# andrew-angus/andvaranaut

Hardware: AMD Instinct MI355X
Metric: gp_lml_evals_per_s (higher is better)
Workload: dtype f64; 1 GPU; Matern52 GP LML eval (assembly + Cholesky + solve), N=16384 d=16, LHS inputs; N=16384, d=16, kernel=Matern52, parallelism=replicas x1 (one chain per GPU)

## Files before the change

andvaranaut_amd/csrc/gemm_f64.hip:

```cpp
#include <cstdlib>
#include <type_traits>
#include "migp_kernels.h"

namespace migp {

typedef double double2_t __attribute__((ext_vector_type(2)));
typedef double double4_t __attribute__((ext_vector_type(4)));

constexpr int TILE = 128;
constexpr int LDS_LD = 144;

__device__ __forceinline__ void tile_from_index(int tri, int nt, int idx, int& ti, int& tj) {
  if (tri) {
    const int ntri = nt * (nt + 1) / 2;
    if (idx < ntri) {
      int t = (int)((sqrt(8.0 * (double)idx + 1.0) - 1.0) * 0.5);
      while ((t + 1) * (t + 2) / 2 <= idx) ++t;
      while (t * (t + 1) / 2 > idx) --t;
      ti = t;
      tj = idx - t * (t + 1) / 2;
    } else {
      const int rem = idx - ntri;
      ti = nt + rem / nt;
      tj = rem % nt;
    }
  } else {
    ti = idx / nt;
    tj = idx % nt;
  }
}
__device__ __forceinline__ void tile_from_index(const GemmParams& p, int idx, int& ti, int& tj) {
  tile_from_index(p.tri, p.nt, idx, ti, tj);
}

__device__ __forceinline__ void tile_from_index_banded(int tri, int mt, int nt, int idx, int R, int& ti, int& tj) {
  auto before = [&](int r) {
    if (!tri) return r * nt;
    return r <= nt ? r * (r + 1) / 2 : nt * (nt + 1) / 2 + (r - nt) * nt;
  };
  int lo = 0, hi = (mt + R - 1) / R - 1;
  while (lo < hi) {
    const int mid = (lo + hi + 1) >> 1;
    if (before(mid * R) <= idx) lo = mid; else hi = mid - 1;
  }
  const int r0 = lo * R, r1 = min(r0 + R, mt), h = r1 - r0;
  int e = idx - before(r0);
  const int cfull = tri ? min(r0 + 1, nt) : nt;
  if (e < cfull * h) { tj = e / h; ti = r0 + e % h; return; }
  e -= cfull * h;
  for (tj = cfull; tj < nt; ++tj) {
    const int cnt = r1 - tj;
    if (e < cnt) { ti = tj + e; return; }
    e -= cnt;
  }
  ti = r1 - 1; tj = min(ti, nt - 1);
}

__device__ __forceinline__ void tile_from_index_banded(const GemmParams& p, int idx, int R, int& ti, int& tj) {
  tile_from_index_banded(p.tri, p.mt, p.nt, idx, R, ti, tj);
}

__device__ __forceinline__ void tile_from_index_fc(int mt, int nt, int fc, int band, int idx, int& ti, int& tj) {
  const int ft = fc * (fc + 1) / 2 + (mt - fc) * fc;
  if (idx < ft) {
    tile_from_index(1, fc, idx, ti, tj);
  } else {
    if (band > 0) tile_from_index_banded(1, mt - fc, nt - fc, idx - ft, band, ti, tj);
    else tile_from_index(1, nt - fc, idx - ft, ti, tj);
    ti += fc;
    tj += fc;
  }
}

__device__ __forceinline__ void list_tile(const GemmParams& p, int idx, int& ra, int& rb, int& rc, int& cc, bool& diag) {
  const int want = idx + p.pl[p.pl_first].x;
  int lo = p.pl_first, hi = p.pl_first + p.pl_n - 1;
  while (lo < hi) {
    const int mid = (lo + hi + 1) >> 1;
    if (p.pl[mid].x <= want) lo = mid; else hi = mid - 1;
  }
  const int4 d = p.pl[lo];
  int ti, tj;
  if (p.band > 0) tile_from_index_banded(1, p.pl_rows - d.y, d.w, want - d.x, p.band, ti, tj);
  else tile_from_index(1, d.w, want - d.x, ti, tj);
  ra = d.y - p.pl_abase + ti;
  rb = d.y - p.pl_abase + tj;
  rc = d.y + ti;
  cc = d.z + tj;
  diag = (ti == tj);
}

namespace vb {
constexpr int BKB = 16;
constexpr int OPER_B = BKB * LDS_LD;
constexpr int NT_B = 256;
constexpr int NQB = TILE * BKB / 2 / NT_B;
#ifndef MIGP_SWZ_B
#define MIGP_SWZ_B 0
#endif
constexpr bool SWZ = MIGP_SWZ_B != 0;

template <bool KMAJOR>
__device__ __forceinline__ void chunk_offsets(long ld, int tid, unsigned& goff, unsigned& loff, long& gstride) {
  if (KMAJOR) {
    const int k = tid >> 6, xc = tid & 63;
    goff = (unsigned)((k * ld + 2 * xc) * 8);
    loff = (unsigned)((k * LDS_LD + 2 * xc) * 8);
    gstride = 4 * ld * 8;
  } else if (SWZ) {
    const int kc = tid & 7, row = tid >> 3;
    goff = (unsigned)((row * ld + 2 * kc) * 8);
    loff = (unsigned)(((2 * kc) * LDS_LD + (row ^ (2 * kc))) * 8);
    gstride = 32 * ld * 8;
  } else {
    const int xl = tid & 15, kc = (tid >> 4) & 7, xh = tid >> 7;
    goff = (unsigned)(((xh * 16 + xl) * ld + 2 * kc) * 8);
    loff = (unsigned)(((2 * kc) * LDS_LD + xh * 16 + xl) * 8);
    gstride = 32 * ld * 8;
  }
}
__device__ __forceinline__ void chunk_load(const char* __restrict__ base, unsigned goff, long gstride,
                                           double2_t (&r)[NQB]) {
#pragma unroll
  for (int q = 0; q < NQB; ++q) r[q] = *reinterpret_cast<const double2_t*>(base + q * gstride + goff);
}
template <bool KMAJOR>
__device__ __forceinline__ void chunk_store(char* __restrict__ lds, unsigned loff, const double2_t (&r)[NQB]) {
#pragma unroll
  for (int q = 0; q < NQB; ++q) {
    if (KMAJOR) {
      *reinterpret_cast<double2_t*>(lds + loff + q * (4 * LDS_LD * 8)) = r[q];
    } else {
      *reinterpret_cast<double*>(lds + loff + q * (32 * 8)) = r[q].x;
      *reinterpret_cast<double*>(lds + loff + q * (32 * 8) + LDS_LD * 8) = r[q].y;
    }
  }
}
}

template <bool A_KMAJOR, bool B_KMAJOR>
__global__ __launch_bounds__(vb::NT_B, 2) void gemm_f64_kernel_b(GemmParams p) {
  using vb::BKB; using vb::OPER_B; using vb::NQB;
  extern __shared__ __attribute__((aligned(16))) double smem[];
  double* As = smem;
  double* Bs = smem + 2 * OPER_B;
  const int tid = threadIdx.x;
  const int lane = tid & 63;
  const int wave = tid >> 6;
  const int wr = wave >> 1, wc = wave & 1;

  const int nblk = gridDim.x;
  int idx = blockIdx.x;
  if (p.kmode == 0) {
    const int b = blockIdx.x, x = b & 7, q = nblk >> 3, r = nblk & 7;
    idx = (x < r ? x * (q + 1) : r * (q + 1) + (x - r) * q) + (b >> 3);
  }
  idx += p.tile0;
  int ti, tj;
  int rc, cc;
  if (p.pl) {
    bool diag;
    list_tile(p, idx, ti, tj, rc, cc, diag);
  } else {
    if (p.fc > 0) tile_from_index_fc(p.mt, p.nt, p.fc, p.band, idx, ti, tj);
    else if (p.band > 0 && p.tri && p.kmode == 0) tile_from_index_banded(p, idx, p.band, ti, tj);
    else tile_from_index(p, idx, ti, tj);
    if (p.kmode == 2 && !p.tri) ti = p.mt - 1 - ti;
    if (p.kmode == 4 && !p.tri) { tj = p.nt - 1 - idx / p.mt; ti = idx % p.mt; }
    rc = ti;
    cc = tj;
  }
  const int i0 = ti * TILE, j0 = tj * TILE;
  int kbeg = 0, kend = p.k;
  if (p.kmode == 1) kbeg = j0;
  else if (p.kmode == 2) kend = i0 + TILE;
  else if (p.kmode == 3) kbeg = i0;
  else if (p.kmode == 4) kend = j0 + TILE;

  const long z1 = p.batch1 > 0 ? (long)(blockIdx.z % p.batch1) : (long)blockIdx.z, z2 = p.batch1 > 0 ? (long)(blockIdx.z / p.batch1) : 0;
  const double* A = p.A + z1 * p.strideA + z2 * p.strideA2;
  const double* B = p.B + z1 * p.strideB + z2 * p.strideB2;
  double* C = p.C + z1 * p.strideC + z2 * p.strideC2;

  double4_t acc[4][4];
#pragma unroll
  for (int a = 0; a < 4; ++a)
#pragma unroll
    for (int b = 0; b < 4; ++b) acc[a][b] = (double4_t){0.0, 0.0, 0.0, 0.0};

  const int nchunk = (kend - kbeg) / BKB;
  unsigned gA, lA, gB, lB;
  long sA, sB;
  vb::chunk_offsets<A_KMAJOR>(p.lda, tid, gA, lA, sA);
  vb::chunk_offsets<B_KMAJOR>(p.ldb, tid, gB, lB, sB);
  const char* Ag = reinterpret_cast<const char*>(A_KMAJOR ? A + (long)kbeg * p.lda + i0 : A + (long)i0 * p.lda + kbeg);
  const char* Bg = reinterpret_cast<const char*>(B_KMAJOR ? B + (long)kbeg * p.ldb + j0 : B + (long)j0 * p.ldb + kbeg);
  const long stepA = (A_KMAJOR ? (long)BKB * p.lda : (long)BKB) * 8;
  const long stepB = (B_KMAJOR ? (long)BKB * p.ldb : (long)BKB) * 8;
  const int segmask = p.kseg > 0 ? p.kseg / BKB - 1 : 0x7fffffff;
  const long segjump = (p.kseg_stride - (long)(p.kseg - BKB)) * 8;
  char* Asb = reinterpret_cast<char*>(As);
  char* Bsb = reinterpret_cast<char*>(Bs);
  double2_t ra[2][NQB], rb[2][NQB];
  if (nchunk > 0) {
    vb::chunk_load(Ag, gA, sA, ra[0]);
    vb::chunk_load(Bg, gB, sB, rb[0]);
    if (nchunk > 1) {
      Ag += stepA;
      Bg += stepB;
      vb::chunk_load(Ag, gA, sA, ra[1]);
      vb::chunk_load(Bg, gB, sB, rb[1]);
    }
    vb::chunk_store<A_KMAJOR>(Asb, lA, ra[0]);
    vb::chunk_store<B_KMAJOR>(Bsb, lB, rb[0]);
  }
  __syncthreads();

  const int kq = lane >> 4, l15 = lane & 15;
  const double* a_ptr[4];
  const double* b_ptr[4];
#pragma unroll
  for (int kk = 0; kk < 4; ++kk) {
    const int sa = (vb::SWZ && !A_KMAJOR) ? (4 * kk + (kq & 2)) : 0, sb = (vb::SWZ && !B_KMAJOR) ? (4 * kk + (kq & 2)) : 0;
    a_ptr[kk] = As + kq * LDS_LD + wr * 64 + (l15 ^ sa);
    b_ptr[kk] = Bs + kq * LDS_LD + wc * 64 + (l15 ^ sb);
  }
  double af[2][4], bf[2][4];
  auto load_frags = [&](int set, int boff, int kk) {
    const double* ap = a_ptr[kk] + boff + kk * 4 * LDS_LD;
    const double* bp = b_ptr[kk] + boff + kk * 4 * LDS_LD;
#pragma unroll
    for (int a = 0; a < 4; ++a) af[set][a] = ap[16 * a];
#pragma unroll
    for (int b = 0; b < 4; ++b) bf[set][b] = bp[16 * b];
  };
  if (nchunk > 0) load_frags(0, 0, 0);

  const double alpha = p.alpha, beta = p.beta;
  double* cbase = C + (long)(rc * TILE + wr * 64 + kq) * p.ldc + cc * TILE + wc * 64 + l15;
  double4_t cv[2][4];
  auto load_group = [&](int set, int a) {
#pragma unroll
    for (int b = 0; b < 4; ++b)
#pragma unroll
      for (int r = 0; r < 4; ++r) cv[set][b][r] = cbase[(long)(16 * a + 4 * r) * p.ldc + 16 * b];
  };
  auto chunk_body = [&](int c, auto S, auto LASTC) {
    constexpr int s = decltype(S)::value;
    constexpr int lastc = decltype(LASTC)::value;
    constexpr int boff = s * OPER_B;
    const bool adv = (c + 2 < nchunk);
    const bool seg = ((c + 2) & segmask) == 0;
    Ag += adv ? (seg ? segjump : stepA) : 0;
    Bg += adv ? (seg ? segjump : stepB) : 0;
#pragma unroll
    for (int kk = 0; kk < BKB / 4; ++kk) {
      const int cur = kk & 1;
      __builtin_amdgcn_sched_barrier(0);
      if (kk == 0) {
        if (lastc == 0) {
          vb::chunk_load(Ag, gA, sA, ra[s]);
          vb::chunk_load(Bg, gB, sB, rb[s]);
        } else {
          load_group(lastc - 1, lastc - 1);
        }
      }
      if (kk + 1 < BKB / 4) load_frags(cur ^ 1, boff, kk + 1);
#pragma unroll
      for (int a = 0; a < 4; ++a)
#pragma unroll
        for (int b = 0; b < 4; ++b)
          acc[a][b] = __builtin_amdgcn_mfma_f64_16x16x4f64(af[cur][a], bf[cur][b], acc[a][b], 0, 0, 0);
      if (kk == BKB / 4 - 1) {
        constexpr int noff = (boff ^ OPER_B) * 8;
        vb::chunk_store<A_KMAJOR>(Asb + noff, lA, ra[s ^ 1]);
        vb::chunk_store<B_KMAJOR>(Bsb + noff, lB, rb[s ^ 1]);
      }
      if (kk == 0) {
#pragma unroll
        for (int g = 0; g < 4; ++g) {
          __builtin_amdgcn_sched_group_barrier(0x008, 1, 0);
          __builtin_amdgcn_sched_group_barrier(0x020, 1, 0);
          __builtin_amdgcn_sched_group_barrier(0x008, 1, 0);
          __builtin_amdgcn_sched_group_barrier(0x020, 1, 0);
          __builtin_amdgcn_sched_group_barrier(0x008, 1, 0);
          __builtin_amdgcn_sched_group_barrier(0x100, 1, 0);
          __builtin_amdgcn_sched_group_barrier(0x008, 1, 0);
        }
      } else if (kk + 1 < BKB / 4) {
#pragma unroll
        for (int g = 0; g < 4; ++g) {
          __builtin_amdgcn_sched_group_barrier(0x008, 3, 0);
          __builtin_amdgcn_sched_group_barrier(0x100, 1, 0);
          __builtin_amdgcn_sched_group_barrier(0x008, 1, 0);
        }
      } else {
        constexpr int nw = (A_KMAJOR ? NQB : 2 * NQB) + (B_KMAJOR ? NQB : 2 * NQB);
#pragma unroll
        for (int g = 0; g < 16; ++g) {
          __builtin_amdgcn_sched_group_barrier(0x008, 1, 0);
          if (g < nw) __builtin_amdgcn_sched_group_barrier(0x200, 1, 0);
        }
      }
    }
    __builtin_amdgcn_sched_barrier(0);
    __syncthreads();
    load_frags(0, boff ^ OPER_B, 0);
  };
  int c = 0;
  for (; c + 2 < nchunk; c += 2) {
    chunk_body(c, std::integral_constant<int, 0>(), std::integral_constant<int, 0>());
    chunk_body(c + 1, std::integral_constant<int, 1>(), std::integral_constant<int, 0>());
  }
  chunk_body(c, std::integral_constant<int, 0>(), std::integral_constant<int, 1>());
  chunk_body(c + 1, std::integral_constant<int, 1>(), std::integral_constant<int, 2>());

  if (beta != 0.0) {
#pragma unroll
    for (int a = 0; a < 4; ++a) {
#pragma unroll
      for (int b = 0; b < 4; ++b)
#pragma unroll
        for (int r = 0; r < 4; ++r)
          cbase[(long)(16 * a + 4 * r) * p.ldc + 16 * b] = alpha * acc[a][b][r] + beta * cv[a & 1][b][r];
      if (a + 2 < 4) load_group(a & 1, a + 2);
    }
  } else {
#pragma unroll
    for (int a = 0; a < 4; ++a)
#pragma unroll
      for (int b = 0; b < 4; ++b)
#pragma unroll
        for (int r = 0; r < 4; ++r) cbase[(long)(16 * a + 4 * r) * p.ldc + 16 * b] = alpha * acc[a][b][r];
  }
}

namespace vs {
constexpr int TS = 64;
constexpr int BKS = 16;
constexpr int LDS_S = 80;
constexpr int OPER_S = BKS * LDS_S;
constexpr int NQS = TS * BKS / 2 / 256;
constexpr int NBUF = 3;
#ifndef MIGP_SWZ_S
#define MIGP_SWZ_S 1
#endif
constexpr bool SWZ = MIGP_SWZ_S != 0;
#ifndef MIGP_XCD_MAP_S
#define MIGP_XCD_MAP_S 1
#endif

template <bool KMAJOR>
__device__ __forceinline__ void chunk_offsets(long ld, int tid, unsigned& goff, unsigned& loff, long& gstride) {
  if (KMAJOR) {
    const int k = tid >> 5, xc = tid & 31;
    goff = (unsigned)((k * ld + 2 * xc) * 8);
    loff = (unsigned)((k * LDS_S + 2 * xc) * 8);
    gstride = 8 * ld * 8;
  } else if (SWZ) {
    const int kc = tid & 7, row = tid >> 3;
    goff = (unsigned)((row * ld + 2 * kc) * 8);
    loff = (unsigned)(((2 * kc) * LDS_S + (row ^ (2 * kc))) * 8);
    gstride = 32 * ld * 8;
  } else {
    const int xl = tid & 15, kc = (tid >> 4) & 7, xh = tid >> 7;
    goff = (unsigned)(((xh * 16 + xl) * ld + 2 * kc) * 8);
    loff = (unsigned)(((2 * kc) * LDS_S + xh * 16 + xl) * 8);
    gstride = 32 * ld * 8;
  }
}
__device__ __forceinline__ void chunk_load(const char* __restrict__ base, unsigned goff, long gstride,
                                           double2_t (&r)[NQS]) {
#pragma unroll
  for (int q = 0; q < NQS; ++q) r[q] = *reinterpret_cast<const double2_t*>(base + q * gstride + goff);
}
template <bool KMAJOR>
__device__ __forceinline__ void chunk_store(char* __restrict__ lds, unsigned loff, const double2_t (&r)[NQS]) {
#pragma unroll
  for (int q = 0; q < NQS; ++q) {
    if (KMAJOR) {
      *reinterpret_cast<double2_t*>(lds + loff + q * (8 * LDS_S * 8)) = r[q];
    } else {
      *reinterpret_cast<double*>(lds + loff + q * (32 * 8)) = r[q].x;
      *reinterpret_cast<double*>(lds + loff + q * (32 * 8) + LDS_S * 8) = r[q].y;
    }
  }
}
}

template <bool A_KMAJOR, bool B_KMAJOR, bool FLUSH = false>
__global__ __launch_bounds__(256, 2) void gemm_f64_kernel_s(GemmParams p) {
  using vs::BKS; using vs::OPER_S; using vs::NQS; using vs::LDS_S; using vs::TS;
  if (p.hiprio) __builtin_amdgcn_s_setprio(3);
  __shared__ __attribute__((aligned(16))) double smem[2 * vs::NBUF * vs::OPER_S];
  double* As = smem;
  double* Bs = smem + vs::NBUF * OPER_S;
  const int tid = threadIdx.x;
  const int lane = tid & 63;
  const int wave = tid >> 6;
  const int wr = wave >> 1, wc = wave & 1;

  int ti, tj;
  int rc, cc;
  int bid = (int)blockIdx.x;
  if (MIGP_XCD_MAP_S && p.kmode == 0) {
    const int nblk = (int)gridDim.x, x = bid & 7, q = nblk >> 3, r = nblk & 7;
    bid = (x < r ? x * (q + 1) : r * (q + 1) + (x - r) * q) + (bid >> 3);
  }
  if (p.pl) {
    int ra, rb, prc, pcc;
    bool diag;
    const int quad = bid & 3;
    list_tile(p, p.sub_base + (bid >> 2), ra, rb, prc, pcc, diag);
    if (diag && quad == 1) return;
    ti = 2 * ra + (quad >> 1);
    tj = 2 * rb + (quad & 1);
    rc = 2 * prc + (quad >> 1);
    cc = 2 * pcc + (quad & 1);
  } else {
    if (p.sub_base >= 0) {
      int pti, ptj;
      const int pidx = p.sub_base + (bid >> 2), quad = bid & 3;
      if (p.fc > 0) tile_from_index_fc(p.sub_mt, p.sub_nt, p.fc, p.band, pidx, pti, ptj);
      else if (p.band > 0 && p.tri) tile_from_index_banded(p.tri, p.sub_mt, p.sub_nt, pidx, p.band, pti, ptj);
      else tile_from_index(p.tri, p.sub_nt, pidx, pti, ptj);
      ti = 2 * pti + (quad >> 1);
      tj = 2 * ptj + (quad & 1);
      if (p.tri && tj > ti) return;
      if (p.dead_last_half && ti == 2 * p.sub_mt - 1) return;
    } else {
      tile_from_index(p, bid, ti, tj);
      if (p.dead_last_half && ti == p.mt - 1) return;
    }
    if (p.kmode == 2 && !p.tri) ti = p.mt - 1 - ti;
    if (p.kmode == 4 && !p.tri) { tj = p.nt - 1 - (int)blockIdx.x / p.mt; ti = (int)blockIdx.x % p.mt; }
    rc = ti;
    cc = tj;
  }
  const int i0 = ti * TS, j0 = tj * TS;
  int kbeg = 0, kend = p.k;
  if (p.kmode == 1) kbeg = j0;
  else if (p.kmode == 2) kend = i0 + TS;
  else if (p.kmode == 3) kbeg = i0;
  else if (p.kmode == 4) kend = j0 + TS;
  kbeg &= ~(BKS - 1);

  const long z1 = p.batch1 > 0 ? (long)(blockIdx.z % p.batch1) : (long)blockIdx.z, z2 = p.batch1 > 0 ? (long)(blockIdx.z / p.batch1) : 0;
  const double* A = p.A + z1 * p.strideA + z2 * p.strideA2;
  const double* B = p.B + z1 * p.strideB + z2 * p.strideB2;
  double* C = p.C + z1 * p.strideC + z2 * p.strideC2;

  double4_t acc[2][2];
#pragma unroll
  for (int a = 0; a < 2; ++a)
#pragma unroll
    for (int b = 0; b < 2; ++b) acc[a][b] = (double4_t){0.0, 0.0, 0.0, 0.0};

  const int nchunk = (kend - kbeg) / BKS;
  unsigned gA, lA, gB, lB;
  long sA, sB;
  vs::chunk_offsets<A_KMAJOR>(p.lda, tid, gA, lA, sA);
  vs::chunk_offsets<B_KMAJOR>(p.ldb, tid, gB, lB, sB);
  const char* Ag = reinterpret_cast<const char*>(A_KMAJOR ? A + (long)kbeg * p.lda + i0 : A + (long)i0 * p.lda + kbeg);
  const char* Bg = reinterpret_cast<const char*>(B_KMAJOR ? B + (long)kbeg * p.ldb + j0 : B + (long)j0 * p.ldb + kbeg);
  const long stepA = (A_KMAJOR ? (long)BKS * p.lda : (long)BKS) * 8;
  const long stepB = (B_KMAJOR ? (long)BKS * p.ldb : (long)BKS) * 8;
  const int segmask = p.kseg > 0 ? p.kseg / BKS - 1 : 0x7fffffff;
  const long segjump = (p.kseg_stride - (long)(p.kseg - BKS)) * 8;
  char* Asb = reinterpret_cast<char*>(As);
  char* Bsb = reinterpret_cast<char*>(Bs);
  constexpr int NB = vs::NBUF;
  double2_t ra[NB][NQS], rb[NB][NQS];
  auto advance = [&](int next_chunk) {
    const bool adv = next_chunk < nchunk;
    const bool seg = (next_chunk & segmask) == 0;
    Ag += adv ? (seg ? segjump : stepA) : 0;
    Bg += adv ? (seg ? segjump : stepB) : 0;
  };
  if (nchunk > 0) {
#pragma unroll
    for (int u = 0; u < NB; ++u) {
      vs::chunk_load(Ag, gA, sA, ra[u]);
      vs::chunk_load(Bg, gB, sB, rb[u]);
      advance(u + 1);
    }
    vs::chunk_store<A_KMAJOR>(Asb, lA, ra[0]);
    vs::chunk_store<B_KMAJOR>(Bsb, lB, rb[0]);
    vs::chunk_store<A_KMAJOR>(Asb + OPER_S * 8, lA, ra[1]);
    vs::chunk_store<B_KMAJOR>(Bsb + OPER_S * 8, lB, rb[1]);
    vs::chunk_load(Ag, gA, sA, ra[0]);
    vs::chunk_load(Bg, gB, sB, rb[0]);
    advance(4);
  }
  const int kq = lane >> 4, l15 = lane & 15;
  const double alpha = p.alpha, beta = p.beta;
  double* cbase = C + (long)(rc * TS + wr * 32 + kq) * p.ldc + cc * TS + wc * 32 + l15;
  double4_t cv[2][2];
  if (beta != 0.0) {
#pragma unroll
    for (int a = 0; a < 2; ++a)
#pragma unroll
      for (int b = 0; b < 2; ++b)
#pragma unroll
        for (int r = 0; r < 4; ++r) cv[a][b][r] = cbase[(long)(16 * a + 4 * r) * p.ldc + 16 * b];
  }
  __syncthreads();

  const double* a_ptr[4];
  const double* b_ptr[4];
#pragma unroll
  for (int kk = 0; kk < 4; ++kk) {
    const int sa = (vs::SWZ && !A_KMAJOR) ? (4 * kk + (kq & 2)) : 0, sb = (vs::SWZ && !B_KMAJOR) ? (4 * kk + (kq & 2)) : 0;
    a_ptr[kk] = As + kq * LDS_S + wr * 32 + (l15 ^ sa);
    b_ptr[kk] = Bs + kq * LDS_S + wc * 32 + (l15 ^ sb);
  }
  double fa[2][2], fb[2][2];
  auto load_frags = [&](int set, int boff, int kk) {
    const double* ap = a_ptr[kk] + boff + kk * 4 * LDS_S;
    const double* bp = b_ptr[kk] + boff + kk * 4 * LDS_S;
    fa[set][0] = ap[0]; fa[set][1] = ap[16]; fb[set][0] = bp[0]; fb[set][1] = bp[16];
  };
  if (nchunk > 0) load_frags(0, 0, 0);
  const int kflush_chunks = FLUSH ? p.kflush / BKS : 1;
  auto chunk_body = [&](int c, auto Sc) {
    constexpr int sidx = decltype(Sc)::value;
    constexpr int boff = sidx * OPER_S;
    constexpr int s1 = (sidx + 1) % NB, s2 = (sidx + 2) % NB;
#pragma unroll
    for (int kk = 0; kk < BKS / 4; ++kk) {
      const int cur = kk & 1;
      __builtin_amdgcn_sched_barrier(0);
      if (kk == 0) {
        vs::chunk_load(Ag, gA, sA, ra[s1]);
        vs::chunk_load(Bg, gB, sB, rb[s1]);
      }
      if (kk + 1 < BKS / 4) load_frags(cur ^ 1, boff, kk + 1);
      else load_frags(cur ^ 1, s1 * OPER_S, 0);
      acc[0][0] = __builtin_amdgcn_mfma_f64_16x16x4f64(fa[cur][0], fb[cur][0], acc[0][0], 0, 0, 0);
      acc[0][1] = __builtin_amdgcn_mfma_f64_16x16x4f64(fa[cur][0], fb[cur][1], acc[0][1], 0, 0, 0);
      acc[1][0] = __builtin_amdgcn_mfma_f64_16x16x4f64(fa[cur][1], fb[cur][0], acc[1][0], 0, 0, 0);
      acc[1][1] = __builtin_amdgcn_mfma_f64_16x16x4f64(fa[cur][1], fb[cur][1], acc[1][1], 0, 0, 0);
      if (kk == BKS / 4 - 1) {
        vs::chunk_store<A_KMAJOR>(Asb + s2 * OPER_S * 8, lA, ra[s2]);
        vs::chunk_store<B_KMAJOR>(Bsb + s2 * OPER_S * 8, lB, rb[s2]);
      }
      if (kk == 0) {
#pragma unroll
        for (int g = 0; g < 2; ++g) {
          __builtin_amdgcn_sched_group_barrier(0x008, 1, 0);
          __builtin_amdgcn_sched_group_barrier(0x020, 1, 0);
          __builtin_amdgcn_sched_group_barrier(0x100, 1, 0);
          __builtin_amdgcn_sched_group_barrier(0x008, 1, 0);
          __builtin_amdgcn_sched_group_barrier(0x020, 1, 0);
        }
      } else if (kk + 1 < BKS / 4) {
#pragma unroll
        for (int g = 0; g < 2; ++g) {
          __builtin_amdgcn_sched_group_barrier(0x008, 1, 0);
          __builtin_amdgcn_sched_group_barrier(0x100, 1, 0);
          __builtin_amdgcn_sched_group_barrier(0x008, 1, 0);
        }
      } else {
#pragma unroll
        for (int g = 0; g < 4; ++g) {
          __builtin_amdgcn_sched_group_barrier(0x008, 1, 0);
          __builtin_amdgcn_sched_group_barrier(0x100, 1, 0);
          __builtin_amdgcn_sched_group_barrier(0x200, 2, 0);
        }
      }
    }
    advance(c + 5);
    __builtin_amdgcn_sched_barrier(0);
    if constexpr (FLUSH) if ((c + 1) % kflush_chunks == 0 && c + 1 < nchunk) {
#pragma unroll
      for (int a = 0; a < 2; ++a)
#pragma unroll
        for (int b = 0; b < 2; ++b) {
#pragma unroll
          for (int r = 0; r < 4; ++r) {
            double v = alpha * acc[a][b][r];
            v += beta * cv[a][b][r];
            cv[a][b][r] = v;
          }
          acc[a][b] = (double4_t){0.0, 0.0, 0.0, 0.0};
        }
    }
    __syncthreads();
  };
  int c = 0;
  for (; c + 3 <= nchunk; c += 3) {
    chunk_body(c, std::integral_constant<int, 0>());
    chunk_body(c + 1, std::integral_constant<int, 1>());
    chunk_body(c + 2, std::integral_constant<int, 2>());
  }
  if (c < nchunk) chunk_body(c, std::integral_constant<int, 0>());
  if (c + 1 < nchunk) chunk_body(c + 1, std::integral_constant<int, 1>());
#pragma unroll
  for (int a = 0; a < 2; ++a)
#pragma unroll
    for (int b = 0; b < 2; ++b)
#pragma unroll
      for (int r = 0; r < 4; ++r) {
        double v = alpha * acc[a][b][r];
        if (beta != 0.0) v += beta * cv[a][b][r];
        cbase[(long)(16 * a + 4 * r) * p.ldc + 16 * b] = v;
      }
}


constexpr size_t LDS_ONE_PER_CU = 82432;

static int tile_count(const GemmParams& p) {
  if (p.pl) return p.pl_tiles;
  if (!p.tri) return p.mt * p.nt;
  return p.nt * (p.nt + 1) / 2 + (p.mt - p.nt) * p.nt;
}


bool gemm_uses_small_tiles(const GemmParams& p, int batch) {
  if (p.kflush > 0) return true;
  return tile_count(p) * batch < p.small_below && p.kmode != 2;
}

constexpr int ROUND_TILES = 512, TAIL_MAX_TILES = 384;
constexpr int NARROW_TRAPEZOID_COLS = 8;
int gemm_tail_tiles(const GemmParams& p, int batch) {
  if (!p.tail_small || p.kmode != 0 || batch != 1 || gemm_uses_small_tiles(p, batch)) return 0;
  const int nblk = tile_count(p), rem = nblk % ROUND_TILES;
  return (nblk > ROUND_TILES && rem > 0 && rem <= TAIL_MAX_TILES) ? rem : 0;
}

hipError_t launch_gemm_f64(const GemmParams& p_in, int opA_kmajor, int opB_kmajor, int batch, hipStream_t stream, int part) {
  GemmParams p = p_in;
  if (p.tri && !p.pl && p.nt <= NARROW_TRAPEZOID_COLS) p.band = 0;
  if (!(p.tri && !p.pl && p.kmode == 0 && p.fc > 0 && p.fc < p.nt)) p.fc = 0;
  if (p.kseg != 0 && (p.kseg < 0 || p.kseg % 128 || p.kmode != 0 || opA_kmajor || opB_kmajor || p.k % p.kseg))
    return hipErrorInvalidValue;
  const int nblk = tile_count(p);
  if (nblk <= 0 || batch <= 0) return hipSuccess;
  const bool small = gemm_uses_small_tiles(p, batch);
  const int tail = gemm_tail_tiles(p, batch);
  auto launch_small = [&](int ntail) -> hipError_t {
    GemmParams q = p;
    q.mt = 2 * p.mt;
    q.nt = 2 * p.nt;
    int nwg = tile_count(q);
    if (ntail > 0) {
      q.sub_base = nblk - ntail;
      q.sub_mt = p.mt;
      q.sub_nt = p.nt;
      nwg = 4 * ntail;
    } else if (p.pl) {
      q.sub_base = 0;
      nwg = 4 * nblk;
    }
    dim3 grid(nwg, 1, batch), block(256);
    const size_t pad = p.one_per_cu ? LDS_ONE_PER_CU - sizeof(double) * 2 * vs::NBUF * vs::OPER_S : 0;
    if (q.kflush > 0) {
      if (opA_kmajor || opB_kmajor || q.kmode != 0 || q.beta == 0.0 || q.kflush % vs::BKS) return hipErrorInvalidValue;
      gemm_f64_kernel_s<false, false, true><<<grid, block, pad, stream>>>(q);
    } else if (!opA_kmajor && !opB_kmajor) gemm_f64_kernel_s<false, false><<<grid, block, pad, stream>>>(q);
    else if (!opA_kmajor && opB_kmajor) gemm_f64_kernel_s<false, true><<<grid, block, pad, stream>>>(q);
    else if (opA_kmajor && opB_kmajor) gemm_f64_kernel_s<true, true><<<grid, block, pad, stream>>>(q);
    else gemm_f64_kernel_s<true, false><<<grid, block, pad, stream>>>(q);
    return hipGetLastError();
  };
  if (small) return (part == 2 || p.tile0 > 0) ? hipSuccess : launch_small(0);
  const int t0 = p.tile0, t1 = p.tile_cnt > 0 ? (t0 + p.tile_cnt < nblk ? t0 + p.tile_cnt : nblk) : nblk;
  const int big_end = t1 < nblk - tail ? t1 : nblk - tail;
  if (part != 2 && big_end > t0) {
    dim3 grid(big_end - t0, 1, batch), block(vb::NT_B);
    const size_t lds = p.one_per_cu ? LDS_ONE_PER_CU : sizeof(double) * 4 * vb::OPER_B;
    if (!opA_kmajor && !opB_kmajor) gemm_f64_kernel_b<false, false><<<grid, block, lds, stream>>>(p);
    else if (!opA_kmajor && opB_kmajor) gemm_f64_kernel_b<false, true><<<grid, block, lds, stream>>>(p);
    else if (opA_kmajor && opB_kmajor) gemm_f64_kernel_b<true, true><<<grid, block, lds, stream>>>(p);
    else gemm_f64_kernel_b<true, false><<<grid, block, lds, stream>>>(p);
    const hipError_t e = hipGetLastError();
    if (e != hipSuccess) return e;
  }
  return (tail > 0 && part != 1 && t1 == nblk) ? launch_small(tail) : hipSuccess;
}

hipError_t gemm_f64_enable_lds() {
  const int ldsb = (int)LDS_ONE_PER_CU;
  hipError_t e = hipFuncSetAttribute(reinterpret_cast<const void*>(gemm_f64_kernel_s<false, false>), hipFuncAttributeMaxDynamicSharedMemorySize, ldsb);
  if (e != hipSuccess) return e;
  e = hipFuncSetAttribute(reinterpret_cast<const void*>(gemm_f64_kernel_s<false, false, true>), hipFuncAttributeMaxDynamicSharedMemorySize, ldsb);
  if (e != hipSuccess) return e;
  e = hipFuncSetAttribute(reinterpret_cast<const void*>(gemm_f64_kernel_s<false, true>), hipFuncAttributeMaxDynamicSharedMemorySize, ldsb);
  if (e != hipSuccess) return e;
  e = hipFuncSetAttribute(reinterpret_cast<const void*>(gemm_f64_kernel_s<true, true>), hipFuncAttributeMaxDynamicSharedMemorySize, ldsb);
  if (e != hipSuccess) return e;
  e = hipFuncSetAttribute(reinterpret_cast<const void*>(gemm_f64_kernel_s<true, false>), hipFuncAttributeMaxDynamicSharedMemorySize, ldsb);
  if (e != hipSuccess) return e;
  e = hipFuncSetAttribute(reinterpret_cast<const void*>(gemm_f64_kernel_b<false, false>), hipFuncAttributeMaxDynamicSharedMemorySize, ldsb);
  if (e != hipSuccess) return e;
  e = hipFuncSetAttribute(reinterpret_cast<const void*>(gemm_f64_kernel_b<false, true>), hipFuncAttributeMaxDynamicSharedMemorySize, ldsb);
  if (e != hipSuccess) return e;
  e = hipFuncSetAttribute(reinterpret_cast<const void*>(gemm_f64_kernel_b<true, true>), hipFuncAttributeMaxDynamicSharedMemorySize, ldsb);
  if (e != hipSuccess) return e;
  return hipFuncSetAttribute(reinterpret_cast<const void*>(gemm_f64_kernel_b<true, false>), hipFuncAttributeMaxDynamicSharedMemorySize, ldsb);
}

}
```

Measured before the change: 40.12 evals/s.

## Use direct global-to-LDS DMA with 4-stage pipeline in f64 GEMM NN path

For the non-transposed A/B case of the big-tile f64 GEMM kernel, operand loads now go straight from global memory into LDS through global_load_lds. This replaces the old path of loading into registers and then storing to LDS. It uses a 4-stage ring buffer with K-chunks of 8, an XOR-swizzled LDS layout, explicit vmcnt waits and re-tuned MFMA scheduling groups. The aim is to free VGPRs and LDS-store instructions and to hide global latency more deeply. In exchange it adds complex hand-counted waitcnt logic, and the swizzle and stage bookkeeping must stay correct. The unused SWZ variant is removed.

After: 40.77 evals/s, median of 6. 1.6% higher.

```diff
diff --git a/andvaranaut_amd/csrc/gemm_f64.hip b/andvaranaut_amd/csrc/gemm_f64.hip
--- a/andvaranaut_amd/csrc/gemm_f64.hip
+++ b/andvaranaut_amd/csrc/gemm_f64.hip
@@ -95,10 +95,6 @@
 constexpr int OPER_B = BKB * LDS_LD;
 constexpr int NT_B = 256;
 constexpr int NQB = TILE * BKB / 2 / NT_B;
-#ifndef MIGP_SWZ_B
-#define MIGP_SWZ_B 0
-#endif
-constexpr bool SWZ = MIGP_SWZ_B != 0;
 
 template <bool KMAJOR>
 __device__ __forceinline__ void chunk_offsets(long ld, int tid, unsigned& goff, unsigned& loff, long& gstride) {
@@ -107,11 +103,6 @@
     goff = (unsigned)((k * ld + 2 * xc) * 8);
     loff = (unsigned)((k * LDS_LD + 2 * xc) * 8);
     gstride = 4 * ld * 8;
-  } else if (SWZ) {
-    const int kc = tid & 7, row = tid >> 3;
-    goff = (unsigned)((row * ld + 2 * kc) * 8);
-    loff = (unsigned)(((2 * kc) * LDS_LD + (row ^ (2 * kc))) * 8);
-    gstride = 32 * ld * 8;
   } else {
     const int xl = tid & 15, kc = (tid >> 4) & 7, xh = tid >> 7;
     goff = (unsigned)(((xh * 16 + xl) * ld + 2 * kc) * 8);
@@ -135,6 +126,35 @@
       *reinterpret_cast<double*>(lds + loff + q * (32 * 8) + LDS_LD * 8) = r[q].y;
     }
   }
+}
+
+constexpr int BKD = 8;
+constexpr int NSTG = 4;
+constexpr int STG_OPER = TILE * BKD * 8;
+constexpr int STG_B = NSTG * STG_OPER;
+constexpr int DMA_PER_CHUNK = 2 * (STG_OPER / (NT_B * 16));
+constexpr size_t LDS_DMA = 2 * NSTG * STG_OPER;
+
+typedef __attribute__((address_space(3))) void* lds_ptr_t;
+typedef __attribute__((address_space(1))) void* gbl_ptr_t;
+
+__device__ __forceinline__ void dma_offsets(long ld, int tid, unsigned& goff, long& gstride) {
+  const int l = tid & 63, w = tid >> 6;
+  const int row = 16 * w + (l >> 2), kp = (l & 3) ^ ((l >> 4) & 3);
+  goff = (unsigned)((row * ld + 2 * kp) * 8);
+  gstride = 64 * ld * 8;
+}
+__device__ __forceinline__ void dma_chunk(const char* __restrict__ g, unsigned goff, long gstride, char* lds_stage, int wave) {
+#pragma unroll
+  for (int q = 0; q < 2; ++q)
+    __builtin_amdgcn_global_load_lds((gbl_ptr_t)(g + q * gstride + goff), (lds_ptr_t)(lds_stage + (4 * q + wave) * 1024), 16, 0, 0);
+}
+template <int N>
+__device__ __forceinline__ void wait_vm() {
+  static_assert(N == 4 || N == 16 || N == 20, "vmcnt");
+  if constexpr (N == 4) asm volatile("s_waitcnt vmcnt(4)" ::: "memory");
+  else if constexpr (N == 16) asm volatile("s_waitcnt vmcnt(16)" ::: "memory");
+  else asm volatile("s_waitcnt vmcnt(20)" ::: "memory");
 }
 }
 
@@ -188,54 +208,8 @@
 #pragma unroll
     for (int b = 0; b < 4; ++b) acc[a][b] = (double4_t){0.0, 0.0, 0.0, 0.0};
 
-  const int nchunk = (kend - kbeg) / BKB;
-  unsigned gA, lA, gB, lB;
-  long sA, sB;
-  vb::chunk_offsets<A_KMAJOR>(p.lda, tid, gA, lA, sA);
-  vb::chunk_offsets<B_KMAJOR>(p.ldb, tid, gB, lB, sB);
-  const char* Ag = reinterpret_cast<const char*>(A_KMAJOR ? A + (long)kbeg * p.lda + i0 : A + (long)i0 * p.lda + kbeg);
-  const char* Bg = reinterpret_cast<const char*>(B_KMAJOR ? B + (long)kbeg * p.ldb + j0 : B + (long)j0 * p.ldb + kbeg);
-  const long stepA = (A_KMAJOR ? (long)BKB * p.lda : (long)BKB) * 8;
-  const long stepB = (B_KMAJOR ? (long)BKB * p.ldb : (long)BKB) * 8;
-  const int segmask = p.kseg > 0 ? p.kseg / BKB - 1 : 0x7fffffff;
-  const long segjump = (p.kseg_stride - (long)(p.kseg - BKB)) * 8;
-  char* Asb = reinterpret_cast<char*>(As);
-  char* Bsb = reinterpret_cast<char*>(Bs);
-  double2_t ra[2][NQB], rb[2][NQB];
-  if (nchunk > 0) {
-    vb::chunk_load(Ag, gA, sA, ra[0]);
-    vb::chunk_load(Bg, gB, sB, rb[0]);
-    if (nchunk > 1) {
-      Ag += stepA;
-      Bg += stepB;
-      vb::chunk_load(Ag, gA, sA, ra[1]);
-      vb::chunk_load(Bg, gB, sB, rb[1]);
-    }
-    vb::chunk_store<A_KMAJOR>(Asb, lA, ra[0]);
-    vb::chunk_store<B_KMAJOR>(Bsb, lB, rb[0]);
-  }
-  __syncthreads();
-
   const int kq = lane >> 4, l15 = lane & 15;
-  const double* a_ptr[4];
-  const double* b_ptr[4];
-#pragma unroll
-  for (int kk = 0; kk < 4; ++kk) {
-    const int sa = (vb::SWZ && !A_KMAJOR) ? (4 * kk + (kq & 2)) : 0, sb = (vb::SWZ && !B_KMAJOR) ? (4 * kk + (kq & 2)) : 0;
-    a_ptr[kk] = As + kq * LDS_LD + wr * 64 + (l15 ^ sa);
-    b_ptr[kk] = Bs + kq * LDS_LD + wc * 64 + (l15 ^ sb);
-  }
   double af[2][4], bf[2][4];
-  auto load_frags = [&](int set, int boff, int kk) {
-    const double* ap = a_ptr[kk] + boff + kk * 4 * LDS_LD;
-    const double* bp = b_ptr[kk] + boff + kk * 4 * LDS_LD;
-#pragma unroll
-    for (int a = 0; a < 4; ++a) af[set][a] = ap[16 * a];
-#pragma unroll
-    for (int b = 0; b < 4; ++b) bf[set][b] = bp[16 * b];
-  };
-  if (nchunk > 0) load_frags(0, 0, 0);
-
   const double alpha = p.alpha, beta = p.beta;
   double* cbase = C + (long)(rc * TILE + wr * 64 + kq) * p.ldc + cc * TILE + wc * 64 + l15;
   double4_t cv[2][4];
@@ -245,75 +219,226 @@
 #pragma unroll
       for (int r = 0; r < 4; ++r) cv[set][b][r] = cbase[(long)(16 * a + 4 * r) * p.ldc + 16 * b];
   };
-  auto chunk_body = [&](int c, auto S, auto LASTC) {
-    constexpr int s = decltype(S)::value;
-    constexpr int lastc = decltype(LASTC)::value;
-    constexpr int boff = s * OPER_B;
-    const bool adv = (c + 2 < nchunk);
-    const bool seg = ((c + 2) & segmask) == 0;
-    Ag += adv ? (seg ? segjump : stepA) : 0;
-    Bg += adv ? (seg ? segjump : stepB) : 0;
-#pragma unroll
-    for (int kk = 0; kk < BKB / 4; ++kk) {
-      const int cur = kk & 1;
-      __builtin_amdgcn_sched_barrier(0);
-      if (kk == 0) {
-        if (lastc == 0) {
-          vb::chunk_load(Ag, gA, sA, ra[s]);
-          vb::chunk_load(Bg, gB, sB, rb[s]);
+  if constexpr (!A_KMAJOR && !B_KMAJOR) {
+    using vb::BKD; using vb::STG_OPER; using vb::STG_B;
+    char* lds = reinterpret_cast<char*>(smem);
+    const int wv = __builtin_amdgcn_readfirstlane(wave);
+    const int nchunk = (kend - kbeg) / BKD;
+    unsigned gA, gB;
+    long sA, sB;
+    vb::dma_offsets(p.lda, tid, gA, sA);
+    vb::dma_offsets(p.ldb, tid, gB, sB);
+    const char* Ag = reinterpret_cast<const char*>(A + (long)i0 * p.lda + kbeg);
+    const char* Bg = reinterpret_cast<const char*>(B + (long)j0 * p.ldb + kbeg);
+    const int segmask = p.kseg > 0 ? p.kseg / BKD - 1 : 0x7fffffff;
+    const long segjump = (p.kseg_stride - (long)(p.kseg - BKD)) * 8;
+    auto advance = [&](int next_chunk) {
+      const long d = (next_chunk & segmask) == 0 ? segjump : (long)BKD * 8;
+      Ag += d;
+      Bg += d;
+    };
+    auto request = [&](int stg) {
+      vb::dma_chunk(Ag, gA, sA, lds + stg * STG_OPER, wv);
+      vb::dma_chunk(Bg, gB, sB, lds + STG_B + stg * STG_OPER, wv);
+    };
+    unsigned foff[2];
+#pragma unroll
+    for (int kk = 0; kk < 2; ++kk) foff[kk] = (unsigned)(l15 * 64 + (((2 * kk + (kq >> 1)) ^ (l15 >> 2)) * 16) + (kq & 1) * 8);
+    const char* a_lds = lds + wr * 64 * 64;
+    const char* b_lds = lds + STG_B + wc * 64 * 64;
+    auto load_frags = [&](int set, int stg, int kk) {
+      const char* ap = a_lds + stg * STG_OPER + foff[kk];
+      const char* bp = b_lds + stg * STG_OPER + foff[kk];
+#pragma unroll
+      for (int a = 0; a < 4; ++a) af[set][a] = *reinterpret_cast<const double*>(ap + 1024 * a);
+#pragma unroll
+      for (int b = 0; b < 4; ++b) bf[set][b] = *reinterpret_cast<const double*>(bp + 1024 * b);
+    };
+    request(0);
+    advance(1);
+    request(1);
+    advance(2);
+    request(2);
+    advance(3);
+    vb::wait_vm<vb::DMA_PER_CHUNK>();
+    __builtin_amdgcn_s_barrier();
+    asm volatile("" ::: "memory");
+    load_frags(0, 0, 0);
+    auto chunk_body = [&](int c, auto S, auto MODE) {
+      constexpr int s = decltype(S)::value;
+      constexpr int mode = decltype(MODE)::value;
+#pragma unroll
+      for (int kk = 0; kk < 2; ++kk) {
+        __builtin_amdgcn_sched_barrier(0);
+        if (kk == 0 && mode <= 1) {
+          request((s + 3) & 3);
+          advance(c + 4);
+        }
+        if (kk == 1 && mode == 1) load_group(0, 0);
+        if (kk == 0 && mode == 3) load_group(1, 1);
+        if (kk == 0) load_frags(1, s, 1);
+        else if (mode != 4) load_frags(0, (s + 1) & 3, 0);
+#pragma unroll
+        for (int a = 0; a < 4; ++a)
+#pragma unroll
+          for (int b = 0; b < 4; ++b)
+            acc[a][b] = __builtin_amdgcn_mfma_f64_16x16x4f64(af[kk][a], bf[kk][b], acc[a][b], 0, 0, 0);
+        if (kk == 0 && mode <= 1) {
+#pragma unroll
+          for (int g = 0; g < 4; ++g) {
+            __builtin_amdgcn_sched_group_barrier(0x008, 1, 0);
+            __builtin_amdgcn_sched_group_barrier(0x020, 1, 0);
+            __builtin_amdgcn_sched_group_barrier(0x008, 1, 0);
+            __builtin_amdgcn_sched_group_barrier(0x100, 2, 0);
+            __builtin_amdgcn_sched_group_barrier(0x008, 2, 0);
+          }
+        } else if (mode == 1 || (kk == 0 && mode == 3)) {
+#pragma unroll
+          for (int g = 0; g < 8; ++g) {
+            __builtin_amdgcn_sched_group_barrier(0x008, 1, 0);
+            __builtin_amdgcn_sched_group_barrier(0x020, 2, 0);
+            __builtin_amdgcn_sched_group_barrier(0x008, 1, 0);
+            __builtin_amdgcn_sched_group_barrier(0x100, 1, 0);
+          }
         } else {
-          load_group(lastc - 1, lastc - 1);
+#pragma unroll
+          for (int g = 0; g < 4; ++g) {
+            __builtin_amdgcn_sched_group_barrier(0x008, 2, 0);
+            __builtin_amdgcn_sched_group_barrier(0x100, 2, 0);
+            __builtin_amdgcn_sched_group_barrier(0x008, 2, 0);
+          }
         }
       }
-      if (kk + 1 < BKB / 4) load_frags(cur ^ 1, boff, kk + 1);
-#pragma unroll
-      for (int a = 0; a < 4; ++a)
-#pragma unroll
-        for (int b = 0; b < 4; ++b)
-          acc[a][b] = __builtin_amdgcn_mfma_f64_16x16x4f64(af[cur][a], bf[cur][b], acc[a][b], 0, 0, 0);
-      if (kk == BKB / 4 - 1) {
-        constexpr int noff = (boff ^ OPER_B) * 8;
-        vb::chunk_store<A_KMAJOR>(Asb + noff, lA, ra[s ^ 1]);
-        vb::chunk_store<B_KMAJOR>(Bsb + noff, lB, rb[s ^ 1]);
+      __builtin_amdgcn_sched_barrier(0);
+      if constexpr (mode <= 2) {
+        vb::wait_vm<mode == 0 ? vb::DMA_PER_CHUNK : mode == 1 ? vb::DMA_PER_CHUNK + 16 : 16>();
+        asm volatile("s_waitcnt lgkmcnt(0)" ::: "memory");
+        __builtin_amdgcn_s_barrier();
+        asm volatile("" ::: "memory");
       }
-      if (kk == 0) {
-#pragma unroll
-        for (int g = 0; g < 4; ++g) {
-          __builtin_amdgcn_sched_group_barrier(0x008, 1, 0);
-          __builtin_amdgcn_sched_group_barrier(0x020, 1, 0);
-          __builtin_amdgcn_sched_group_barrier(0x008, 1, 0);
-          __builtin_amdgcn_sched_group_barrier(0x020, 1, 0);
-          __builtin_amdgcn_sched_group_barrier(0x008, 1, 0);
-          __builtin_amdgcn_sched_group_barrier(0x100, 1, 0);
-          __builtin_amdgcn_sched_group_barrier(0x008, 1, 0);
+    };
+    int c = 0;
+    for (; c + 4 < nchunk; c += 4) {
+      chunk_body(c, std::integral_constant<int, 0>(), std::integral_constant<int, 0>());
+      chunk_body(c + 1, std::integral_constant<int, 1>(), std::integral_constant<int, 0>());
+      chunk_body(c + 2, std::integral_constant<int, 2>(), std::integral_constant<int, 0>());
+      chunk_body(c + 3, std::integral_constant<int, 3>(), std::integral_constant<int, 0>());
+    }
+    chunk_body(c, std::integral_constant<int, 0>(), std::integral_constant<int, 1>());
+    chunk_body(c + 1, std::integral_constant<int, 1>(), std::integral_constant<int, 2>());
+    chunk_body(c + 2, std::integral_constant<int, 2>(), std::integral_constant<int, 3>());
+    chunk_body(c + 3, std::integral_constant<int, 3>(), std::integral_constant<int, 4>());
+  } else {
+    const int nchunk = (kend - kbeg) / BKB;
+    unsigned gA, lA, gB, lB;
+    long sA, sB;
+    vb::chunk_offsets<A_KMAJOR>(p.lda, tid, gA, lA, sA);
+    vb::chunk_offsets<B_KMAJOR>(p.ldb, tid, gB, lB, sB);
+    const char* Ag = reinterpret_cast<const char*>(A_KMAJOR ? A + (long)kbeg * p.lda + i0 : A + (long)i0 * p.lda + kbeg);
+    const char* Bg = reinterpret_cast<const char*>(B_KMAJOR ? B + (long)kbeg * p.ldb + j0 : B + (long)j0 * p.ldb + kbeg);
+    const long stepA = (A_KMAJOR ? (long)BKB * p.lda : (long)BKB) * 8;
+    const long stepB = (B_KMAJOR ? (long)BKB * p.ldb : (long)BKB) * 8;
+    const int segmask = p.kseg > 0 ? p.kseg / BKB - 1 : 0x7fffffff;
+    const long segjump = (p.kseg_stride - (long)(p.kseg - BKB)) * 8;
+    char* Asb = reinterpret_cast<char*>(As);
+    char* Bsb = reinterpret_cast<char*>(Bs);
+    double2_t ra[2][NQB], rb[2][NQB];
+    if (nchunk > 0) {
+      vb::chunk_load(Ag, gA, sA, ra[0]);
+      vb::chunk_load(Bg, gB, sB, rb[0]);
+      if (nchunk > 1) {
+        Ag += stepA;
+        Bg += stepB;
+        vb::chunk_load(Ag, gA, sA, ra[1]);
+        vb::chunk_load(Bg, gB, sB, rb[1]);
+      }
+      vb::chunk_store<A_KMAJOR>(Asb, lA, ra[0]);
+      vb::chunk_store<B_KMAJOR>(Bsb, lB, rb[0]);
+    }
+    __syncthreads();
+
+    const double* a_ptr = As + kq * LDS_LD + wr * 64 + l15;
+    const double* b_ptr = Bs + kq * LDS_LD + wc * 64 + l15;
+    auto load_frags = [&](int set, int boff, int kk) {
+      const double* ap = a_ptr + boff + kk * 4 * LDS_LD;
+      const double* bp = b_ptr + boff + kk * 4 * LDS_LD;
+  #pragma unroll
+      for (int a = 0; a < 4; ++a) af[set][a] = ap[16 * a];
+  #pragma unroll
+      for (int b = 0; b < 4; ++b) bf[set][b] = bp[16 * b];
+    };
+    if (nchunk > 0) load_frags(0, 0, 0);
+
+    auto chunk_body = [&](int c, auto S, auto LASTC) {
+      constexpr int s = decltype(S)::value;
+      constexpr int lastc = decltype(LASTC)::value;
+      constexpr int boff = s * OPER_B;
+      const bool adv = (c + 2 < nchunk);
+      const bool seg = ((c + 2) & segmask) == 0;
+      Ag += adv ? (seg ? segjump : stepA) : 0;
+      Bg += adv ? (seg ? segjump : stepB) : 0;
+  #pragma unroll
+      for (int kk = 0; kk < BKB / 4; ++kk) {
+        const int cur = kk & 1;
+        __builtin_amdgcn_sched_barrier(0);
+        if (kk == 0) {
+          if (lastc == 0) {
+            vb::chunk_load(Ag, gA, sA, ra[s]);
+            vb::chunk_load(Bg, gB, sB, rb[s]);
+          } else {
+            load_group(lastc - 1, lastc - 1);
+          }
         }
-      } else if (kk + 1 < BKB / 4) {
-#pragma unroll
-        for (int g = 0; g < 4; ++g) {
-          __builtin_amdgcn_sched_group_barrier(0x008, 3, 0);
-          __builtin_amdgcn_sched_group_barrier(0x100, 1, 0);
-          __builtin_amdgcn_sched_group_barrier(0x008, 1, 0);
+        if (kk + 1 < BKB / 4) load_frags(cur ^ 1, boff, kk + 1);
+  #pragma unroll
+        for (int a = 0; a < 4; ++a)
+  #pragma unroll
+          for (int b = 0; b < 4; ++b)
+            acc[a][b] = __builtin_amdgcn_mfma_f64_16x16x4f64(af[cur][a], bf[cur][b], acc[a][b], 0, 0, 0);
+        if (kk == BKB / 4 - 1) {
+          constexpr int noff = (boff ^ OPER_B) * 8;
+          vb::chunk_store<A_KMAJOR>(Asb + noff, lA, ra[s ^ 1]);
+          vb::chunk_store<B_KMAJOR>(Bsb + noff, lB, rb[s ^ 1]);
         }
-      } else {
-        constexpr int nw = (A_KMAJOR ? NQB : 2 * NQB) + (B_KMAJOR ? NQB : 2 * NQB);
-#pragma unroll
-        for (int g = 0; g < 16; ++g) {
-          __builtin_amdgcn_sched_group_barrier(0x008, 1, 0);
-          if (g < nw) __builtin_amdgcn_sched_group_barrier(0x200, 1, 0);
+        if (kk == 0) {
+  #pragma unroll
+          for (int g = 0; g < 4; ++g) {
+            __builtin_amdgcn_sched_group_barrier(0x008, 1, 0);
+            __builtin_amdgcn_sched_group_barrier(0x020, 1, 0);
+            __builtin_amdgcn_sched_group_barrier(0x008, 1, 0);
+            __builtin_amdgcn_sched_group_barrier(0x020, 1, 0);
+            __builtin_amdgcn_sched_group_barrier(0x008, 1, 0);
+            __builtin_amdgcn_sched_group_barrier(0x100, 1, 0);
+            __builtin_amdgcn_sched_group_barrier(0x008, 1, 0);
+          }
+        } else if (kk + 1 < BKB / 4) {
+  #pragma unroll
+          for (int g = 0; g < 4; ++g) {
+            __builtin_amdgcn_sched_group_barrier(0x008, 3, 0);
+            __builtin_amdgcn_sched_group_barrier(0x100, 1, 0);
+            __builtin_amdgcn_sched_group_barrier(0x008, 1, 0);
+          }
+        } else {
+          constexpr int nw = (A_KMAJOR ? NQB : 2 * NQB) + (B_KMAJOR ? NQB : 2 * NQB);
+  #pragma unroll
+          for (int g = 0; g < 16; ++g) {
+            __builtin_amdgcn_sched_group_barrier(0x008, 1, 0);
+            if (g < nw) __builtin_amdgcn_sched_group_barrier(0x200, 1, 0);
+          }
         }
       }
-    }
-    __builtin_amdgcn_sched_barrier(0);
-    __syncthreads();
-    load_frags(0, boff ^ OPER_B, 0);
-  };
-  int c = 0;
-  for (; c + 2 < nchunk; c += 2) {
-    chunk_body(c, std::integral_constant<int, 0>(), std::integral_constant<int, 0>());
-    chunk_body(c + 1, std::integral_constant<int, 1>(), std::integral_constant<int, 0>());
-  }
-  chunk_body(c, std::integral_constant<int, 0>(), std::integral_constant<int, 1>());
-  chunk_body(c + 1, std::integral_constant<int, 1>(), std::integral_constant<int, 2>());
+      __builtin_amdgcn_sched_barrier(0);
+      __syncthreads();
+      load_frags(0, boff ^ OPER_B, 0);
+    };
+    int c = 0;
+    for (; c + 2 < nchunk; c += 2) {
+      chunk_body(c, std::integral_constant<int, 0>(), std::integral_constant<int, 0>());
+      chunk_body(c + 1, std::integral_constant<int, 1>(), std::integral_constant<int, 0>());
+    }
+    chunk_body(c, std::integral_constant<int, 0>(), std::integral_constant<int, 1>());
+    chunk_body(c + 1, std::integral_constant<int, 1>(), std::integral_constant<int, 2>());
+  }
 
   if (beta != 0.0) {
 #pragma unroll
@@ -670,7 +795,8 @@
   const int big_end = t1 < nblk - tail ? t1 : nblk - tail;
   if (part != 2 && big_end > t0) {
     dim3 grid(big_end - t0, 1, batch), block(vb::NT_B);
-    const size_t lds = p.one_per_cu ? LDS_ONE_PER_CU : sizeof(double) * 4 * vb::OPER_B;
+    const bool dma = !opA_kmajor && !opB_kmajor;
+    const size_t lds = p.one_per_cu ? LDS_ONE_PER_CU : dma ? vb::LDS_DMA : sizeof(double) * 4 * vb::OPER_B;
     if (!opA_kmajor && !opB_kmajor) gemm_f64_kernel_b<false, false><<<grid, block, lds, stream>>>(p);
     else if (!opA_kmajor && opB_kmajor) gemm_f64_kernel_b<false, true><<<grid, block, lds, stream>>>(p);
     else if (opA_kmajor && opB_kmajor) gemm_f64_kernel_b<true, true><<<grid, block, lds, stream>>>(p);
```
